# phylo42/IPK

Measured on AMD Instinct MI355X. Metric: scored phylo-k-mers/sec, higher is better.
Workload: dtype f32

## Files before the change

ipk_amd/csrc/ipkgpu.hip:

```cpp
#include <cstring>
#include <hip/hip_runtime.h>
#include <rocprim/rocprim.hpp>

#include <algorithm>
#include <cmath>
#include <cstdarg>
#include <cstdio>
#include <cstring>
#include <new>
#include <string>
#include <type_traits>
#include <unordered_map>
#include <memory>
#include <vector>

#include "../../include/ipkgpu.h"
#include "dcla_device.hpp"
#include "kernels_score.hpp"
#include "kernels_quad.hpp"
#include "kernels_compact.hpp"
#include "kernels_keymajor.hpp"
#include "kernels_reduce_pipe.hpp"
#include "kernels_filter.hpp"
#include "kernels_dbfile.hpp"
// ... 39 lines not shown
        if (!e) return -1;
        (void)hipEventRecord(e, stream);
        ev.push_back(e);
        return (int)ev.size() - 1;
    }
    double ms(int a, int b) const
    {
        float t = 0;
        if (a < 0 || b < 0 || hipEventElapsedTime(&t, ev[a], ev[b]) != hipSuccess) return 0;
        return t;
    }
};

}

struct ipkgpu_comm;
struct ipkgpu_ctx;
static void ipkgpu_comm_release(ipkgpu_ctx* ctx);
struct ipkgpu_ctx {
    int device = 0;
    ipkgpu_comm* comm = nullptr;
    hipStream_t stream = nullptr;
    std::string err;
    int64_t workspace_bytes = 0;
    int64_t opt_variant = 0;
    int64_t opt_flags = 0;
    int64_t opt_kmc_pass = 0;
    int64_t opt_slice = 0;
    uint64_t sliced_windows = 0;
    int64_t opt_prefix_mats = 0;
    int64_t opt_wg_chunks2 = 0;
    int64_t opt_rounds = 0;
    int64_t opt_pool_limit = 0;
    int64_t opt_pool_chunks = 0;
    DevBuf table, best, ovfq, counts, offsets, goff, idx, branch, scan_sums, scan_boff, tmp_a, tmp_b, tmp_c;
    DevBuf pool, desc, gbcnt, gboff, gbcur, clist, gm, tile_next;
    DevBuf ptrs;
    DevBuf sp_bits, sp_pops, sp_rank, sp_c16;
    void* h_spill[2] = {nullptr, nullptr}; hipEvent_t ev_spill[2] = {nullptr, nullptr}; size_t h_spill_cap = 0;
    size_t held = 0, held_peak = 0;
    int64_t budget = 0;
    size_t refused_need = 0;
    DevBuf mask;
    bool mask_valid = false;
    uint64_t mask_words = 0;
    bool table_compressed = false;
    DevBuf rank, vaddr, ucnt, qpack, xstart, pcounts;
    DevBuf seq, pvals, pvaddr, mrank, cursnap;
    DevBuf cvals, coff, croom;
    bool comp_own_vals = false;
    std::vector<uint32_t> h_branch;
    uint32_t comp_nb = 0, comp_stride = 0, comp_tbl = 0;
    double pairs_per_window = 0;
    double acc_main_ms = 0, acc_reduce_ms = 0;
    double acc_count_ms = 0, acc_write_ms = 0, acc_km_ms = 0;
    const char* main_kernel = "";
    std::vector<std::pair<void*, size_t>> free_blocks;
    std::unordered_map<void*, size_t> live_blocks;
    size_t cached_bytes = 0, cache_limit = 0;
    void* small = nullptr;
    void* h_up = nullptr; size_t h_up_cap = 0; hipEvent_t up_done = nullptr; bool up_pending = false;
    unsigned long long emitted_host = 0; bool emitted_fetched = false;
    uint32_t* h_rb = nullptr;
    EventPool events;
    bool spec_skip_wait = false;
    uint64_t pool_want_min = 0;
    struct Pending {
        bool active = false;
        std::unique_ptr<Stopwatch> sw; int ev_a = -1, ev_b = -1, ev_c = -1, ev_d = -1;
        uint64_t cap = 0, max_chunks = 0, windows = 0; uint32_t gb = 0; bool pool_ovf_ok = false, use_quad = false;
    } pend;
    uint64_t last_entries = 0; uint32_t last_gb = 0;
    double t_write_total = 0, t_write_device = 0, t_write_file = 0;
    int64_t opt_load_chunk = 0;
    double t_load[8] = {0, 0, 0, 0, 0, 0, 0, 0};
    double t_diff_ms = 0;
    DevBuf place_seq, place_off, place_out, place_tables, place_small, place_amb;
    int64_t opt_place_batch = 0;
    int64_t opt_place_lds = 0;
    int num_cu = 256;
};

struct ipkgpu_result {
    ipkgpu_ctx* ctx = nullptr;
    std::vector<uint32_t> group_ids;
    std::vector<uint64_t> offsets;
    uint64_t emitted = 0;
    uint32_t* d_keys = nullptr;
    float* d_scores = nullptr;
    uint32_t* d_positions = nullptr;
    size_t cap = 0;
    std::vector<uint32_t> h_keys;
    std::vector<float> h_scores;
    std::vector<uint32_t> h_positions;
    bool h_keys_ok = false, h_scores_ok = false, h_positions_ok = false;
    double t_total = 0, t_prefix = 0, t_score = 0, t_compact = 0, t_main = 0, t_reduce = 0;
    int score_launches = 0;
};

struct ipkgpu_parts {
    ipkgpu_ctx* ctx = nullptr;
    uint32_t n_owners = 1;
    uint64_t slots = 0;
    uint32_t* d_counts = nullptr;
    uint2* d_entries = nullptr;
    uint32_t* d_positions = nullptr;
// ... 1134 lines not shown
    p.mask = ctx->mask.as<uint32_t>(); p.mask_words = ctx->mask_words;
    if (ps.kind == PassKind::xp) {
        if (!ps.compress) {
            RC_TRY(ensure(ctx, ctx->table, (size_t)gb * pl.table_size * 4));
            p.table = ctx->table.p;
        }
        const int rc = score_batch_xp(ctx, pl, logp_dev, gb, p);
        return rc ? rc : check_capped(ctx, pl.k, p);
    }

    const bool pool_ovf_ok = gb < (1u << 22) && n_mats < (1u << 21) && pl.nwin < (1u << 21);
    bool s_compress = pool_ovf_ok && ps.compress;
    const uint32_t NBK = pl.geo.stream_nb, TBL = pl.geo.stream_tbl;
    const uint32_t SNW = use_quad ? pl.geo.quad_nw : pl.geo.stream_nw;
    const uint32_t STW = use_quad ? pl.geo.quad_tw : pl.geo.stream_tw;
    const uint32_t s_tiles_per_mat = (pl.nwin + STW - 1) / STW;
    auto pass1 = [&](const StreamParams& sp, uint32_t n_wg, bool count_only) {
        return with_sigma_k(ctx, pl.sigma, pl.k, [&](auto S_, auto K_) {
            if (!use_quad) return launch_stream_pass1<S_, K_>(ctx, sp, n_wg);
            return count_only ? launch_quad_pass1<S_, K_, true>(ctx, sp, n_wg, ps.layout) : launch_quad_pass1<S_, K_, false>(ctx, sp, n_wg, ps.layout);
        });
    };

    const uint64_t windows = (uint64_t)nb * pl.nwin;
    if (ctx->pairs_per_window <= 0) {
        const uint32_t n_s = std::min<uint32_t>(gb, std::max<uint32_t>(2, gb / 64));
        const uint32_t stride_g = gb / n_s;
        std::vector<uint32_t> sgm((size_t)n_s + 1, 0), slist;
        for (uint32_t j = 0; j < n_s; ++j) {
            const uint32_t g = j * stride_g;
            for (uint32_t m = gm[g]; m < gm[g + 1]; ++m) slist.push_back(gm[(size_t)gb + 1 + m]);
            sgm[j + 1] = (uint32_t)slist.size();
        }
        std::vector<uint32_t> both(sgm);
        both.insert(both.end(), slist.begin(), slist.end());
        RC_TRY(ensure(ctx, ctx->tmp_a, both.size() * 4));
        HIP_TRY(ctx, hipMemcpyAsync(ctx->tmp_a.p, both.data(), both.size() * 4, hipMemcpyHostToDevice, ctx->stream));
        HIP_TRY(ctx, hipMemsetAsync(p.emitted, 0, 8, ctx->stream));
        HIP_TRY(ctx, hipMemsetAsync(p.ovf_count, 0, 4, ctx->stream));
        StreamParams ss;
        ss.logp = logp_dev; ss.best = ctx->best.as<float>();
        ss.gm_off = ctx->tmp_a.as<uint32_t>(); ss.gm_list = ctx->tmp_a.as<uint32_t>() + n_s + 1;
        ss.sites = pl.sites; ss.nwin = pl.nwin; ss.tiles_per_mat = s_tiles_per_mat;
        ss.S = (uint32_t)std::max<uint64_t>(1, std::min<uint64_t>(s_tiles_per_mat, (uint64_t)ctx->num_cu * 4 / n_s));
        ss.eps = pl.eps;
        ss.pool = nullptr; ss.pool_cap = 0; ss.pool_next = nullptr; ss.desc = nullptr; ss.pool_ovf = nullptr; ss.pre_chunks = 0;
        ss.emitted = p.emitted; ss.ovf_queue = p.ovf_queue; ss.ovf_count = p.ovf_count; ss.mat_slot = p.mat_slot;
        ss.flags = 2u;
        RC_TRY(pass1(ss, n_s * ss.S, true));
        unsigned long long se = 0; uint32_t so = 0;
        HIP_TRY(ctx, hipMemcpyAsync(&se, p.emitted, 8, hipMemcpyDeviceToHost, ctx->stream));
        HIP_TRY(ctx, hipMemcpyAsync(&so, p.ovf_count, 4, hipMemcpyDeviceToHost, ctx->stream));
        HIP_TRY(ctx, hipStreamSynchronize(ctx->stream));
        const uint64_t s_windows = (uint64_t)slist.size() * pl.nwin;
        const double cap_pairs = 0.25 * (double)pl.geo.fast_cap * (double)pl.geo.fast_cap;
        if (s_windows) ctx->pairs_per_window = std::max(1.0, ((double)se + (double)so * cap_pairs) / (double)s_windows * 1.15);
    }
    const double ppw_est = ctx->pairs_per_window > 0 ? ctx->pairs_per_window : 256.0;
    if (!s_compress && pool_ovf_ok && ctx->opt_variant == 0 && pl.table_size >= (1u << 16) &&
        (double)windows * ppw_est < 0.5 * (double)gb * (double)pl.table_size)
        s_compress = true;
    if (!s_compress) {
        RC_TRY(ensure(ctx, ctx->table, (size_t)gb * pl.table_size * 4));
        p.table = ctx->table.p;
    }
    const size_t lds_bytes = use_quad ? pl.geo.quad_lds : pl.geo.stream_lds;
    const uint64_t wg_per_cu = std::max<uint64_t>(1, std::min<uint64_t>(32 / SNW, (160 * 1024) / std::max<size_t>(lds_bytes, 1)));
    const uint64_t slots = (uint64_t)ctx->num_cu * wg_per_cu;
    const uint32_t CH = chunk_pairs_rt(TBL);
    const uint64_t CHB = chunk_bytes_rt(TBL, ps.layout);
    const uint64_t expected_chunks = (uint64_t)((double)windows * ppw_est / CH);
#ifndef IPK_WG_CHUNKS2
#define IPK_WG_CHUNKS2 2
#endif
    const uint64_t wg_chunks2 = ctx->opt_wg_chunks2 > 0 ? (uint64_t)ctx->opt_wg_chunks2 : (uint64_t)IPK_WG_CHUNKS2;
    const uint64_t max_wg = std::max<uint64_t>(slots, expected_chunks * 2 / wg_chunks2 / ((uint64_t)SNW * NBK * SUB));
#ifndef IPK_ROUNDS
#define IPK_ROUNDS 8
#endif
    const uint64_t rounds = std::max<uint64_t>(1, std::min<uint64_t>(ctx->opt_rounds > 0 ? (uint64_t)ctx->opt_rounds : (uint64_t)IPK_ROUNDS, max_wg / slots));
    uint64_t S64 = std::max<uint64_t>(1, (slots * rounds) / gb);
    uint32_t S = (uint32_t)std::max<uint64_t>(1, std::min<uint64_t>(S64, s_tiles_per_mat));
    const uint32_t n_wg = gb * S;
    const uint64_t n_waves = (uint64_t)n_wg * SNW;
    const uint64_t n_gb = (uint64_t)gb * NBK;

    const size_t free_b = mem_free_bytes(ctx);
    uint64_t max_chunks = std::min<uint64_t>(0xFFFFFFF0ull, (uint64_t)(free_b + ctx->pool.cap + ctx->desc.cap) * 9 / 10 / (CHB + 8));
    if (ctx->opt_pool_limit > 0) max_chunks = std::min<uint64_t>(max_chunks, (uint64_t)ctx->opt_pool_limit / (CHB + 8));
    const double ppw = ctx->pairs_per_window > 0 ? ctx->pairs_per_window : 256.0;
    const uint64_t ovf_waves = (uint64_t)ctx->num_cu * 4 * OVF_NW;
    const uint64_t slack = 2 * (n_waves + ovf_waves) * NBK * SUB + (n_waves + ovf_waves) * ALLOC_BATCH + 1024;
    uint64_t want = (uint64_t)((double)windows * ppw * 1.25 / CH) + slack;
    {
        const uint64_t have = std::min<uint64_t>(std::max<uint64_t>(ctx->pool.cap / CHB, 1) - 1, ctx->desc.cap / 8);
        const uint64_t need = (uint64_t)((double)windows * ppw * 1.1 / CH) + (n_waves + ovf_waves) * (NBK * SUB + ALLOC_BATCH) + 1024;
        if (have >= need) want = have;
    }
    want = std::max<uint64_t>(want, ctx->pool_want_min);
    for (int attempt = 0; attempt < 6; ++attempt) {
        uint64_t cap = std::min<uint64_t>(want, max_chunks);
        const bool forced = attempt == 0 && ctx->opt_pool_chunks > 0 && ctx->pool_want_min == 0;
        if (forced) cap = (uint64_t)ctx->opt_pool_chunks;
        else if (cap < n_waves * NBK * SUB) {
            if (gb > 1) return IPKGPU_RETRY_SMALLER;
            return fail(ctx, IPKGPU_ERR_NOMEM, "the pair pool of ONE branch group does not fit device memory");
// ... 1476 lines not shown

std::string spill_block_path(const char* dir, uint32_t piece, uint32_t owner)
{
    char name[64];
    snprintf(name, sizeof name, "/p%u_b%u.blk", piece, owner);
    return std::string(dir) + name;
}

struct SpillFile {
    std::string path; ipkspill::Head head; uint64_t key_base = 0, entry_base = 0;
};

int spill_check_files(ipkgpu_ctx* ctx, uint32_t sigma, uint32_t k, uint32_t owner, uint32_t n_owners, const char* const* paths, uint32_t n_blocks,
                      uint64_t slots, std::vector<SpillFile>& files)
{
    files.resize(n_blocks);
    uint64_t keys = 0, entries = 0;
    for (uint32_t s = 0; s < n_blocks; ++s) {
        if (!paths[s]) return fail(ctx, IPKGPU_ERR_INVALID, "null path of block %u", s);
        SpillFile& f = files[s];
        f.path = paths[s];
        FILE* fh = fopen(paths[s], "rb");
        if (!fh) return fail(ctx, IPKGPU_ERR_INVALID, "cannot open spill block %s", paths[s]);
        struct stat st;
        const bool stat_ok = fstat(fileno(fh), &st) == 0;
        memset(&f.head, 0, sizeof f.head);
        const size_t got = fread(&f.head, 1, sizeof f.head, fh);
        fclose(fh);
        if (!stat_ok) return fail(ctx, IPKGPU_ERR_INVALID, "cannot stat spill block %s", paths[s]);
        const char* what = got < sizeof f.head ? "shorter than a block's head"
                                               : ipkspill::check_head(f.head, (uint64_t)st.st_size, sigma, k, n_owners, owner, slots);
        if (what) return fail(ctx, IPKGPU_ERR_INVALID, "spill block %s: %s", paths[s], what);
        f.key_base = keys; f.entry_base = entries;
        keys += f.head.n_keys; entries += f.head.n_entries;
    }
    return IPKGPU_OK;
}

}

extern "C" {

int ipkgpu_get_option(const ipkgpu_ctx* ctx, const char* name, int64_t* value)
{
    if (!ctx || !name || !value) return IPKGPU_ERR_INVALID;
    if (!strcmp(name, "workspace_bytes")) { *value = ctx->workspace_bytes; return IPKGPU_OK; }
    if (!strcmp(name, "device_budget_bytes")) { *value = ctx->budget; return IPKGPU_OK; }
    if (!strcmp(name, "last_refused_bytes")) { *value = (int64_t)ctx->refused_need; return IPKGPU_OK; }
    if (!strcmp(name, "slice_long_lists")) { *value = ctx->opt_slice; return IPKGPU_OK; }
    if (!strcmp(name, "db_load_chunk_bytes")) { *value = ctx->opt_load_chunk; return IPKGPU_OK; }
    if (!strcmp(name, "place_batch_queries")) { *value = ctx->opt_place_batch; return IPKGPU_OK; }
    if (!strcmp(name, "place_lds_branches")) { *value = ctx->opt_place_lds; return IPKGPU_OK; }
    if (!strcmp(name, "debug_sliced_windows")) { *value = (int64_t)ctx->sliced_windows; return IPKGPU_OK; }
    if (!strcmp(name, "debug_pool_bytes")) { *value = (int64_t)ctx->pool.cap; return IPKGPU_OK; }
    return IPKGPU_ERR_INVALID;
}

int ipkgpu_mem_stats(ipkgpu_ctx* ctx, uint64_t* held, uint64_t* held_peak, int reset_peak)
{
    if (!ctx) return IPKGPU_ERR_INVALID;
    if (held) *held = ctx->held;
    if (held_peak) *held_peak = ctx->held_peak;
    if (reset_peak) ctx->held_peak = ctx->held;
    return IPKGPU_OK;
}

int ipkgpu_parts_spill(ipkgpu_ctx* ctx, ipkgpu_parts* parts, const char* dir, uint32_t piece, uint64_t* bytes_written)
{
    if (!ctx) return IPKGPU_ERR_INVALID;
    if (!parts || parts->ctx != ctx || !dir) return fail(ctx, IPKGPU_ERR_INVALID, "bad argument");
    if (parts->d_positions) return fail(ctx, IPKGPU_ERR_INVALID, "positioned parts are not spilled: the on-disk build keeps no positions (as the reference's, db_builder.cpp:469)");
    if (parts->lead != 0) return fail(ctx, IPKGPU_ERR_INVALID, "key-range parts are not spilled: a key-range pass already bounds the device");
    if (!parts->d_counts || !parts->d_entries) return fail(ctx, IPKGPU_ERR_INVALID, "these parts' arrays have moved into a database");
    HIP_TRY(ctx, hipSetDevice(ctx->device));
    const uint32_t B = parts->n_owners;
    const uint64_t slots = parts->slots, W = ipkspill::bit_words(slots), n_words = (uint64_t)B * W;
    if (W > 0xFFFFFFFFull || (n_words + 3) / 4 > 0x7FFFFFFFull) return fail(ctx, IPKGPU_ERR_INVALID, "too many key slots to spill");
    RC_TRY(ensure(ctx, ctx->sp_bits, n_words * 8));
    RC_TRY(ensure(ctx, ctx->sp_pops, n_words * 4));
    RC_TRY(ensure(ctx, ctx->sp_rank, (n_words + 1) * 8));
    RC_TRY(ensure(ctx, ctx->goff, ((size_t)B + 1) * 8));
    uint32_t* d_big = small_at(ctx, SMALL_REC_BIG);
    HIP_TRY(ctx, hipMemsetAsync(d_big, 0, 4, ctx->stream));
    const uint32_t grid = (uint32_t)((n_words + 3) / 4);
    hipLaunchKernelGGL(spill_bits_kernel, dim3(grid), dim3(256), 0, ctx->stream, parts->d_counts, slots, W, n_words,
                       ctx->sp_bits.as<unsigned long long>(), ctx->sp_pops.as<uint32_t>(), d_big);
    HIP_TRY(ctx, hipGetLastError());
    RC_TRY(scan_u32(ctx, ctx->sp_pops.as<uint32_t>(), n_words, ctx->sp_rank.as<uint64_t>()));
    hipLaunchKernelGGL(gather_offsets_kernel, dim3((B + 1 + 255) / 256), dim3(256), 0, ctx->stream, ctx->sp_rank.as<uint64_t>(), (uint32_t)W, B + 1,
                       ctx->goff.as<uint64_t>());
    HIP_TRY(ctx, hipGetLastError());
    std::vector<uint64_t> key_base((size_t)B + 1);
    uint32_t h_big = 0;
    HIP_TRY(ctx, hipMemcpyAsync(key_base.data(), ctx->goff.p, ((size_t)B + 1) * 8, hipMemcpyDeviceToHost, ctx->stream));
    HIP_TRY(ctx, hipMemcpyAsync(&h_big, d_big, 4, hipMemcpyDeviceToHost, ctx->stream));
    HIP_TRY(ctx, hipStreamSynchronize(ctx->stream));
    if (h_big) return fail(ctx, IPKGPU_ERR_INVALID, "a key with more than %u entries in one piece: a spill block's counts are 16-bit (pieces of at most %u groups)",
                           ipkspill::COUNT_MAX, ipkspill::COUNT_MAX);
    RC_TRY(ensure(ctx, ctx->sp_c16, key_base[B] * 2));
    hipLaunchKernelGGL(spill_pack_kernel, dim3(grid), dim3(256), 0, ctx->stream, parts->d_counts, slots, W, n_words, ctx->sp_rank.as<uint64_t>(),
                       ctx->sp_c16.as<uint16_t>());
    HIP_TRY(ctx, hipGetLastError());

    uint64_t largest = 0;
    for (uint32_t o = 0; o < B; ++o)
        largest = std::max(largest, ipkspill::file_bytes(slots, key_base[o + 1] - key_base[o], parts->owner_off[o + 1] - parts->owner_off[o]));
// ... 163 lines not shown
```

ipk_amd/csrc/kernels_quad.hpp:

```cpp
#pragma once
#include "kernels_score.hpp"

namespace ipkgpu {

struct QuadNode { int J, H, TH, OFF; uint32_t F, CMUL; };
struct QuadStep { int H, A, B; };

template <int SIGMA, int K>
struct QuadGeo {
    using D = HalvesDD<SIGMA, K>;
    static constexpr int HL = D::HL, HR = D::HR, LA = D::LA, LB = D::LB, RA = D::RA, RB = D::RB;
    static constexpr bool OK = SIGMA == 4 && D::OK && LA >= 2 && LA <= 3 && LB >= 2 && LB <= 3 && RA >= 2 && RA <= 3 && RB >= 2 && RB <= 3;
    static constexpr uint32_t FLA = D::FLA, FLB = D::FLB, FRA = D::FRA, FRB = D::FRB;
    static constexpr uint32_t mulR = ipow(SIGMA, K - K / 2);
    static constexpr uint32_t CW = FLA + FLB + FRA + FRB;
    static constexpr int th_n(int h) { return h == 2 ? 3 : 5; }
    static constexpr int TH0 = 2, TH1 = TH0 + th_n(LA), TH2 = TH1 + th_n(LB), TH3 = TH2 + th_n(RA);
    static constexpr int TH_F = TH3 + th_n(RB);
    static constexpr int PADW = 1;
    static constexpr QuadNode node(int n)
    {
        return n == 0 ? QuadNode{0, LA, TH0, 0, FLA, 1u}
             : n == 1 ? QuadNode{LA, LB, TH1, (int)FLA, FLB, mulR}
             : n == 2 ? QuadNode{HL, RA, TH2, (int)(FLA + FLB), FRA, 1u}
                      : QuadNode{HL + RA, RB, TH3, (int)(FLA + FLB + FRA), FRB, 1u};
    }
    static constexpr int count_h(int h) { int c = 0; for (int n = 0; n < 4; ++n) c += node(n).H == h; return c; }
    static constexpr int nth_h(int h, int i) { for (int n = 0; n < 4; ++n) if (node(n).H == h) { if (i == 0) return n; --i; } return -1; }
    static constexpr int NS2 = (count_h(2) + 1) / 2, NS3 = (count_h(3) + 1) / 2, NSTEPS = NS2 + NS3;
    static constexpr QuadStep step(int s)
    {
        return s < NS2 ? QuadStep{2, nth_h(2, 2 * s), nth_h(2, 2 * s + 1)} : QuadStep{3, nth_h(3, 2 * (s - NS2)), nth_h(3, 2 * (s - NS2) + 1)};
    }
    static constexpr int step_of(int n) { for (int s = 0; s < NSTEPS; ++s) if (step(s).A == n || step(s).B == n) return s; return -1; }
    static constexpr int slot_of(int n) { return step(step_of(n)).B == n ? 1 : 0; }
    static constexpr int NS1 = (count_h(2) > 0 ? 1 : 0) + (count_h(3) > 0 ? 1 : 0);
    static constexpr int step1_h(int s) { return (s == 0 && count_h(2) > 0) ? 2 : 3; }
    static constexpr int step1_node(int s, int slot) { return nth_h(step1_h(s), slot); }
    static constexpr int step1_of(int n) { return node(n).H == 2 ? 0 : (count_h(2) > 0 ? 1 : 0); }
    static constexpr int slot1_of(int n) { int c = 0; for (int m = 0; m < n; ++m) c += node(m).H == node(n).H; return c; }
};

template <int SIGMA, int K, int TW>
struct QuadTile {
    static constexpr int TC = TW + K - 1 + QuadGeo<SIGMA, K>::PADW;
    static constexpr int COLS_F = TC * SIGMA;
    static constexpr int BEST_F = ((TC + 1 + 3) / 4) * 4;
    static constexpr int TH_FLOATS = (((TW + QuadGeo<SIGMA, K>::PADW) * QuadGeo<SIGMA, K>::TH_F + 3) / 4) * 4;
    static constexpr int HEAD_BYTES = (COLS_F + BEST_F + TH_FLOATS) * 4;
};

template <int SIGMA, int K, int CAP, bool ONEWIN = false>
constexpr uint32_t quad_wave_entries()
{
    using Q = QuadGeo<SIGMA, K>;
    return (ONEWIN ? 1 : 2) * Q::CW + Geo<SIGMA, Q::HL, CAP>::CAPH + Geo<SIGMA, Q::HR, CAP>::CAPH;
}

template <int J, int H>
__device__ __forceinline__ void quad_node_thresholds(const float* bs, float e, float* out)
{
    out[0] = e;
    if constexpr (H == 2) {
        out[1] = e - (bs[J + 2] - bs[J + 1]);
        out[2] = e - (bs[J + 1] - bs[J]);
    } else {
        static_assert(H == 3, "child nodes have 2 or 3 symbols");
        const float e_leaf = e - (bs[J + 3] - bs[J + 1]);
        const float e_pair = e - (bs[J + 1] - bs[J]);
        out[1] = e_leaf;
        out[2] = e_pair;
        out[3] = e_pair - (bs[J + 3] - bs[J + 2]);
        out[4] = e_pair - (bs[J + 2] - bs[J + 1]);
    }
}

template <int H>
__device__ __forceinline__ void quad_step(const float* cols, uint32_t base, bool valid, uint64_t vmask, const float* th, uint2* list,
                                          uint32_t l16, uint32_t slot, uint32_t lt16, uint32_t code16, uint32_t cmul, uint32_t& count)
{
    const float e = th[0];
    if constexpr (H == 2) {
        const float sl = cols[base + (l16 >> 2)], sr = cols[base + 4 + (l16 & 3u)];
        const float s = sl + sr;
        const bool c1 = sl > th[1], c2 = sr > th[2], c3 = s > e;
        const bool pass = valid & c1 & c2 & c3;
        const uint64_t m = vmask & ballot64(c1) & ballot64(c2) & ballot64(c3);
        const uint32_t x = (uint32_t)(m >> (16u * slot));
        const uint32_t pos = (uint32_t)__popc(x & lt16);
        if (pass) list[pos] = make_uint2(code16, __float_as_uint(s));
        count = (uint32_t)__popc(x & 0xFFFFu);
    } else {
        const float sj = cols[base + 4 + (l16 >> 2)], sl2 = cols[base + 8 + (l16 & 3u)];
        const float s2 = sj + sl2;
        const bool d1 = sj > th[3], d2 = sl2 > th[4], d3 = s2 > th[2];
        const bool okp = valid & d1 & d2 & d3;
        const uint64_t mp = vmask & ballot64(d1) & ballot64(d2) & ballot64(d3);
        uint32_t run = 0;
#pragma unroll
        for (int i = 0; i < 4; ++i) {
            const float si = cols[base + i];
            const float s = si + s2;
            const bool c1 = si > th[1], c2 = s > e;
            const bool pass = okp & c1 & c2;
            const uint64_t m = mp & ballot64(c1) & ballot64(c2);
            const uint32_t x = (uint32_t)(m >> (16u * slot));
            const uint32_t pos = (uint32_t)__popc(x & lt16) + run;
            if (pass) list[pos] = make_uint2(__umul24(cmul, (uint32_t)i * 16u) + code16, __float_as_uint(s));
            run += (uint32_t)__popc(x & 0xFFFFu);
        }
        count = run;
    }
}

__device__ __forceinline__ void pool_store(uint2* wave_base, uint32_t byte_off, uint2 val)
{
    const unsigned long long data = ((unsigned long long)val.y << 32) | val.x;
    asm volatile("global_store_dwordx2 %0, %1, %2" : : "v"(byte_off), "v"(data), "s"(wave_base) : "memory");
}
__device__ __forceinline__ uint32_t lshl3_add(uint32_t x, uint32_t y)
{
    uint32_t r;
    asm("v_lshl_add_u32 %0, %1, 3, %2" : "=v"(r) : "v"(x), "v"(y));
    return r;
}
__device__ __forceinline__ void pool_store_lanes(uint2* wave_base, uint32_t byte_off, uint2 val, uint64_t mask)
{
    const unsigned long long data = ((unsigned long long)val.y << 32) | val.x;
    IPK_ASSERT_FULL_EXEC();
    asm volatile("s_mov_b64 exec, %3\n\tglobal_store_dwordx2 %0, %1, %2\n\ts_mov_b64 exec, -1"
                 : : "v"(byte_off), "v"(data), "s"(wave_base), "s"(mask) : "memory");
}

__device__ __forceinline__ uint64_t pool_store_inside(uint2* wave_base, uint32_t byte_off, uint2 val, uint32_t v, uint64_t pass, uint32_t CH)
{
    const unsigned long long data = ((unsigned long long)val.y << 32) | val.x;
    uint64_t outside;
    IPK_ASSERT_FULL_EXEC();
    asm volatile("s_mov_b64 exec, %5\n\t"
                 "v_cmpx_gt_u32_e32 vcc, %6, %4\n\t"
                 "global_store_dwordx2 %1, %2, %3\n\t"
                 "s_andn2_b64 %0, %5, exec\n\t"
                 "s_mov_b64 exec, -1"
                 : "=&s"(outside) : "v"(byte_off), "v"(data), "s"(wave_base), "v"(v), "s"(pass), "s"(CH) : "memory", "vcc");
    return outside;
}


template <uint32_t SLOT_PLANE>
__device__ __forceinline__ void pool_store6(uint2* wave_base, uint32_t off4, uint32_t off2, uint2 val)
{
    static_assert(SLOT_PLANE < 4096, "the slot plane's offset must fit the store's immediate field");
    asm volatile("global_store_dword %0, %2, %4\n\tglobal_store_short %1, %3, %4 offset:%5"
                 : : "v"(off4), "v"(off2), "v"(val.y), "v"(val.x), "s"(wave_base), "n"(SLOT_PLANE) : "memory");
}
template <int SH>
__device__ __forceinline__ uint32_t lshl_add(uint32_t x, uint32_t y)
{
    uint32_t r;
    asm("v_lshl_add_u32 %0, %1, %3, %2" : "=v"(r) : "v"(x), "v"(y), "n"(SH));
    return r;
}
template <uint32_t SLOT_PLANE>
__device__ __forceinline__ uint64_t pool_store_inside6(uint2* wave_base, uint32_t off4, uint32_t off2, uint2 val, uint32_t v, uint64_t pass, uint32_t CH)
{
    static_assert(SLOT_PLANE < 4096, "the slot plane's offset must fit the store's immediate field");
    uint64_t outside;
    IPK_ASSERT_FULL_EXEC();
    asm volatile("s_mov_b64 exec, %7\n\t"
                 "v_cmpx_gt_u32_e32 vcc, %8, %6\n\t"
                 "global_store_dword %1, %3, %5\n\t"
                 "global_store_short %2, %4, %5 offset:%9\n\t"
                 "s_andn2_b64 %0, %7, exec\n\t"
                 "s_mov_b64 exec, -1"
                 : "=&s"(outside) : "v"(off4), "v"(off2), "v"(val.y), "v"(val.x), "s"(wave_base), "v"(v), "s"(pass), "s"(CH), "n"(SLOT_PLANE)
                 : "memory", "vcc");
    return outside;
// ... 92 lines not shown
    __device__ __forceinline__ void init(uint32_t wave_gid)
    {
        const uint32_t first = wave_gid * NB;
        const bool pre = p.pre_chunks != 0 && first + NB <= p.pre_chunks && first + NB <= p.pool_cap;
        for (uint32_t b = lane_id(); b < NB; b += 64)
            st[b] = pre ? ((unsigned long long)(first + b) << 32) : (((unsigned long long)NONE << 32) | (unsigned long long)CH);
    }
    __device__ __forceinline__ uint32_t roll_at(uint32_t b, uint32_t x)
    {
        const uint32_t lane = lane_id();
        if (chunk_next == chunk_end) {
            uint32_t first = 0;
            if (lane == 0) first = atomicAdd(p.pool_next, ALLOC_BATCH);
            chunk_next = (uint32_t)__builtin_amdgcn_readfirstlane((int)first);
            chunk_end = chunk_next + ALLOC_BATCH;
        }
        uint32_t nid = to_sgpr(chunk_next);
        chunk_next = nid + 1;
        if (nid >= p.pool_cap && lane == 0) atomicOr(p.pool_ovf, 1u);
        nid = min(nid, p.pool_cap);
        wave_lds_sync();
        const unsigned long long old = st[b];
        wave_lds_sync();
        if (lane == 0) {
            const uint32_t oid = (uint32_t)(old >> 32);
            if (oid < p.pool_cap) p.desc[oid] = ((unsigned long long)(g * NB + b) << 32) | (unsigned long long)x;
            st[b] = ((unsigned long long)nid << 32) | (unsigned long long)((uint32_t)old - x);
        }
        wave_lds_sync();
        return nid;
    }
    __device__ __forceinline__ void close()
    {
        wave_lds_sync();
        for (uint32_t b = lane_id(); b < NB; b += 64) {
            const unsigned long long s = st[b];
            const uint32_t id = (uint32_t)(s >> 32);
            if (id < p.pool_cap) p.desc[id] = ((unsigned long long)(g * NB + b) << 32) | (unsigned long long)min((uint32_t)s, CH);
        }
    }
};

__device__ __forceinline__ void store_pair_if_gt(unsigned long long& cursor, uint32_t x, float s, float eps)
{
    u32x2_t data; data.x = x; data.y = __float_as_uint(s);
    IPK_ASSERT_FULL_EXEC();
    asm volatile("v_cmpx_lt_f32_e32 vcc, %3, %2\n\t"
                 "global_store_dwordx2 %0, %1, off\n\t"
                 "v_lshl_add_u64 %0, %0, 0, 8\n\t"
                 "s_mov_b64 exec, -1"
                 : "+v"(cursor) : "v"(data), "v"(s), "s"(eps) : "vcc");
}

template <uint32_t MUL>
__device__ __forceinline__ uint32_t half_join_single(const uint2* A, const uint2* B, uint32_t nb, uint32_t total, float eps, uint2* out,
                                                     uint32_t lane, float lane_h)
{
    const float rn = __builtin_amdgcn_rcpf((float)nb);
    const uint32_t i = div_small(lane_h, rn), j = (uint32_t)(__mul24((int)i, -(int)nb) + (int)lane);
    const uint2 a = A[i], b = B[j];
    const float s = __uint_as_float(a.y) + __uint_as_float(b.y);
    const bool v = lane < total, c = s > eps;
    const uint64_t h = ballot64(v) & ballot64(c);
    if (v && c) out[mbcnt(h)] = make_uint2(a.x * MUL + b.x, __float_as_uint(s));
    return (uint32_t)__popcll(h);
}
template <uint32_t MUL>
__device__ __forceinline__ uint32_t half_join_rows(const uint2* A, uint32_t na, const uint2* B, uint32_t nb, float eps, uint2* out, uint32_t cap,
                                                   uint32_t lane, float lane_h)
{
    const float rn = __builtin_amdgcn_rcpf((float)nb);
    const uint32_t rps = to_sgpr(div_small(64.5f, rn));
    const uint32_t rsel = div_small(lane_h, rn), col = lane - __umul24(rsel, nb);
    const uint2 b = B[col];
    const float by = __uint_as_float(b.y);
    const uint2* ap = A + rsel;
    uint32_t n = 0;
    for (uint32_t i0 = 0; i0 < na; i0 += rps) {
        const uint2 a = ap[i0];
        const float s = __uint_as_float(a.y) + by;
        const bool live = lane < min(rps, na - i0) * nb, c = s > eps;
        const uint64_t m = ballot64(live) & ballot64(c);
        const uint32_t cnt = (uint32_t)__popcll(m);
        if (n + cnt > cap) return LIST_OVERFLOW;
        if (live && c) (out + n)[mbcnt(m)] = make_uint2(a.x * MUL + b.x, __float_as_uint(s));
        n += cnt;
    }
    return n;
}

template <int SIGMA, int K, int CAP, int TW, int NW, uint32_t TBL, bool COUNT_ONLY = false, bool ROWLANE = false, bool ONEWIN = false,
          PairLayout LAYOUT = PairLayout::PAIR8>
__global__ __launch_bounds__(NW * 64) void score_quad_kernel(StreamParams p)
{
    extern __shared__ __align__(16) unsigned char smem[];
    using Q = QuadGeo<SIGMA, K>;
    using QT = QuadTile<SIGMA, K, TW>;
    static_assert(Q::OK, "quad kernel: DNA k = 8..12");
    constexpr uint32_t T = ipow(SIGMA, K);
    constexpr uint32_t NB = (T + TBL - 1) / TBL;
    constexpr uint32_t CH = chunk_pairs<TBL>();
    constexpr uint32_t mulR = Q::mulR;
    static_assert(TBL % mulR == 0, "a row of the final join must stay inside one bucket");
    using CL = ChunkLayout<TBL, LAYOUT>;
    static_assert(!ROWLANE || LAYOUT == PairLayout::PAIR8, "the row-per-lane join writes 8-byte pairs");
    constexpr bool P6 = LAYOUT == PairLayout::PAIR6;
    constexpr uint32_t CAPL = Geo<SIGMA, Q::HL, CAP>::CAPH, CAPR = Geo<SIGMA, Q::HR, CAP>::CAPH;
    constexpr uint32_t WS = quad_wave_entries<SIGMA, K, CAP, ONEWIN>();
    constexpr uint32_t WPW = ONEWIN ? 1u : 2u;
    constexpr int NST = ONEWIN ? Q::NS1 : Q::NSTEPS;
    float* cols = reinterpret_cast<float*>(smem);
    float* best = cols + QT::COLS_F;
    float* thr = best + QT::BEST_F;
    uint2* scratch_all = reinterpret_cast<uint2*>(smem + QT::HEAD_BYTES);
    unsigned long long* state_all = reinterpret_cast<unsigned long long*>(scratch_all + (size_t)NW * WS);

    const uint32_t lane = lane_id();
    const uint32_t wave = (uint32_t)__builtin_amdgcn_readfirstlane((int)(threadIdx.x >> 6));
    const uint32_t g = blockIdx.x / p.S, seg = blockIdx.x - g * p.S;
    const uint32_t m0 = p.gm_off[g], nm = p.gm_off[g + 1] - m0;
    const uint32_t total_tiles = nm * p.tiles_per_mat;
    const uint32_t t_lo = (uint32_t)(((uint64_t)total_tiles * seg) / p.S);
    const uint32_t t_hi = (uint32_t)(((uint64_t)total_tiles * (seg + 1)) / p.S);

    uint2* child = scratch_all + (size_t)wave * WS;
    uint2* lp = child + WPW * Q::CW;
    uint2* rp = lp + CAPL;
    using Appender = std::conditional_t<ROWLANE, LaneAppender<NB, CH>, RowAppender<NB, CH, CL::PAIR_BYTES>>;
    Appender app{p, state_all + (size_t)wave * NB, g};
    app.init(blockIdx.x * NW + wave);
    unsigned long long emitted = 0;

    const uint32_t l16 = lane & 15u, slot = lane >> 4, half = ONEWIN ? 0u : lane >> 5, sb = slot & 1u;
    const uint32_t lt16 = (1u << l16) - 1u;
    const float lane_h = (float)lane + 0.5f;
    const float eps = p.eps;
    constexpr bool count_only = COUNT_ONLY;
    uint32_t st_j4[NST], st_th[NST], st_off[NST], st_cmul[NST], st_code[NST];
    bool st_on[NST];
#pragma unroll
    for (int s = 0; s < NST; ++s) {
        constexpr QuadNode none{0, 2, 0, 0, 0, 1u};
        if constexpr (ONEWIN) {
            QuadNode nd = none;
            bool on = false;
#pragma unroll
            for (int sl = 0; sl < 4; ++sl) {
                const int n = Q::step1_node(s, sl);
                if (n >= 0 && slot == (uint32_t)sl) { nd = Q::node(n); on = true; }
            }
            st_j4[s] = (uint32_t)nd.J * 4u; st_th[s] = (uint32_t)nd.TH; st_off[s] = (uint32_t)nd.OFF; st_cmul[s] = nd.CMUL;
            st_code[s] = l16 * st_cmul[s]; st_on[s] = on;
        } else {
            const QuadStep qs = Q::step(s);
            const QuadNode na = Q::node(qs.A), nb = qs.B >= 0 ? Q::node(qs.B) : none;
            st_j4[s] = sb ? (uint32_t)nb.J * 4u : (uint32_t)na.J * 4u;
            st_th[s] = sb ? (uint32_t)nb.TH : (uint32_t)na.TH;
            st_off[s] = (sb ? (uint32_t)nb.OFF : (uint32_t)na.OFF) + half * Q::CW;
            st_cmul[s] = sb ? nb.CMUL : na.CMUL;
            st_code[s] = l16 * st_cmul[s];
            st_on[s] = sb ? qs.B >= 0 : true;
        }
    }

    __shared__ uint32_t sh_tile;
    const bool draw = p.tile_next != nullptr;
    uint32_t t = t_lo, t_end = t_hi;
    if (draw) { t = seg; t_end = total_tiles; }
    while (t < t_end) {
        const uint32_t q = t / p.tiles_per_mat, tile = t - q * p.tiles_per_mat;
        const uint32_t mat = p.gm_list[m0 + q];
        const uint32_t t0 = tile * TW;
        const uint32_t nw = min((uint32_t)TW, p.nwin - t0);
        const uint32_t ncol = nw + K - 1;
        __syncthreads();
        uint32_t t_drawn = 0;
        if (draw && threadIdx.x == 0) t_drawn = atomicAdd(&p.tile_next[g], 1u);
        {
            const float4* src = reinterpret_cast<const float4*>(p.logp + ((size_t)mat * p.sites + t0) * SIGMA);
            float4* dst = reinterpret_cast<float4*>(cols);
            const uint32_t n4 = ncol * (SIGMA / 4);
            for (uint32_t i = threadIdx.x; i < n4; i += NW * 64) dst[i] = src[i];
            const float* bsrc = p.best + (size_t)mat * (p.sites + 1) + t0;
            for (uint32_t i = threadIdx.x; i <= ncol; i += NW * 64) best[i] = bsrc[i];
        }
        if (draw && threadIdx.x == 0) sh_tile = t_drawn;
        __syncthreads();
        for (uint32_t w = threadIdx.x; w < nw; w += NW * 64) {
            const float* bs = best + w;
            float* o = thr + w * Q::TH_F;
            const float eps_l = eps - (bs[K] - bs[Q::HL]);
            const float eps_r = eps - (bs[Q::HL] - bs[0]);
            o[0] = eps_l; o[1] = eps_r;
            quad_node_thresholds<0, Q::LA>(bs, eps_l - (bs[Q::HL] - bs[Q::LA]), o + Q::node(0).TH);
            quad_node_thresholds<Q::LA, Q::LB>(bs, eps_l - (bs[Q::LA] - bs[0]), o + Q::node(1).TH);
            quad_node_thresholds<Q::HL, Q::RA>(bs, eps_r - (bs[K] - bs[Q::HL + Q::RA]), o + Q::node(2).TH);
            quad_node_thresholds<Q::HL + Q::RA, Q::RB>(bs, eps_r - (bs[Q::HL + Q::RA] - bs[Q::HL]), o + Q::node(3).TH);
        }
        __syncthreads();

        const uint32_t npair = (nw + WPW - 1) / WPW;
        const float* thw = thr + __umul24(wave * WPW + half, (uint32_t)Q::TH_F);
        for (uint32_t pr = wave; pr < npair; pr += NW, thw += WPW * NW * Q::TH_F) {
            const uint32_t wq = pr * WPW;
            const uint32_t wl = wq + half;
            const bool wvalid = wl < nw;
            uint32_t counts[3] = {0, 0, 0};
            wave_lds_sync();
            auto run_step = [&](auto S) {
                constexpr int s = decltype(S)::value;
                if constexpr (s < NST) {
                    const bool valid = wvalid && st_on[s];
                    const uint64_t vmask = ballot64(valid);
                    const uint32_t base = wl * 4 + st_j4[s];
                    constexpr int H = ONEWIN ? Q::step1_h(s) : Q::step(s < Q::NSTEPS ? s : 0).H;
                    quad_step<H>(cols, base, valid, vmask, thw + st_th[s], child + st_off[s], l16, slot, lt16, st_code[s], st_cmul[s], counts[s]);
                }
            };
            run_step(std::integral_constant<int, 0>{});
            run_step(std::integral_constant<int, 1>{});
            run_step(std::integral_constant<int, 2>{});
            wave_lds_sync();
            const uint32_t nwp = min(WPW, nw - wq);

#pragma unroll 1
            for (uint32_t gw = 0; gw < nwp; ++gw) {
                const uint32_t w = wq + gw;
                constexpr int so0 = ONEWIN ? Q::step1_of(0) : Q::step_of(0), so1 = ONEWIN ? Q::step1_of(1) : Q::step_of(1);
                constexpr int so2 = ONEWIN ? Q::step1_of(2) : Q::step_of(2), so3 = ONEWIN ? Q::step1_of(3) : Q::step_of(3);
                constexpr int sl0 = ONEWIN ? Q::slot1_of(0) : Q::slot_of(0), sl1 = ONEWIN ? Q::slot1_of(1) : Q::slot_of(1);
                constexpr int sl2 = ONEWIN ? Q::slot1_of(2) : Q::slot_of(2), sl3 = ONEWIN ? Q::slot1_of(3) : Q::slot_of(3);
                const uint32_t wbase = ONEWIN ? 0u : gw * 32u;
                const uint32_t nla = (uint32_t)__builtin_amdgcn_readlane((int)counts[so0], (int)(wbase + sl0 * 16));
                const uint32_t nlb = (uint32_t)__builtin_amdgcn_readlane((int)counts[so1], (int)(wbase + sl1 * 16));
                const uint32_t nra = (uint32_t)__builtin_amdgcn_readlane((int)counts[so2], (int)(wbase + sl2 * 16));
                const uint32_t nrb = (uint32_t)__builtin_amdgcn_readlane((int)counts[so3], (int)(wbase + sl3 * 16));
                if (nla * nlb * nra * nrb == 0) continue;
                const uint2* cw = child + gw * Q::CW;
                const uint2 *la = cw + Q::node(0).OFF, *lb = cw + Q::node(1).OFF, *ra = cw + Q::node(2).OFF, *rb = cw + Q::node(3).OFF;
                const float eps_l = thr[w * Q::TH_F], eps_r = thr[w * Q::TH_F + 1];
                const uint32_t tl = nla * nlb, tr = nra * nrb;
                uint32_t nL, nR;
                constexpr bool SLICE = ROWLANE;
                constexpr uint32_t SAFE_L = CAPL / Q::FLB, SAFE_R = CAPR / Q::FRB;
                static_assert(SAFE_L >= 1 && SAFE_R >= 1, "a slice of one row of the first child must fit the list");
                const bool one_step = tl <= 64 && tr <= 64;
                uint32_t sla = nla, sra = nra, ia = 0, ir = 0;
                bool keep_l = false;
                for (;;) {
                wave_lds_sync();
                if (one_step) {
                    const float rnl = __builtin_amdgcn_rcpf((float)nlb), rnr = __builtin_amdgcn_rcpf((float)nrb);
                    const uint32_t il = div_small(lane_h, rnl), jl = (uint32_t)(__mul24((int)il, -(int)nlb) + (int)lane);
                    const uint32_t ir = div_small(lane_h, rnr), jr = (uint32_t)(__mul24((int)ir, -(int)nrb) + (int)lane);
                    const uint2 a0 = la[il], b0 = lb[jl], a1 = ra[ir], b1 = rb[jr];
                    const float s0 = __uint_as_float(a0.y) + __uint_as_float(b0.y);
                    const float s1 = __uint_as_float(a1.y) + __uint_as_float(b1.y);
                    const bool v0 = lane < tl, v1 = lane < tr, c0 = s0 > eps_l, c1 = s1 > eps_r;
                    const bool p0 = v0 && c0, p1 = v1 && c1;
                    const uint64_t h0 = ballot64(v0) & ballot64(c0), h1 = ballot64(v1) & ballot64(c1);
                    if (p0) lp[mbcnt(h0)] = make_uint2(a0.x * (Q::FLB * mulR) + b0.x, __float_as_uint(s0));
                    if (p1) rp[mbcnt(h1)] = make_uint2(a1.x * Q::FRB + b1.x, __float_as_uint(s1));
                    nL = (uint32_t)__popcll(h0); nR = (uint32_t)__popcll(h1);
                } else {
                    if constexpr (!ROWLANE) {
                        nL = (uint32_t)__builtin_amdgcn_readfirstlane((int)(tl <= 64 ? half_join_single<Q::FLB * mulR>(la, lb, nlb, tl, eps_l, lp, lane, lane_h)
                                                                                       : half_join_rows<Q::FLB * mulR>(la, nla, lb, nlb, eps_l, lp, CAPL, lane, lane_h)));
                        nR = nL == LIST_OVERFLOW || nL == 0 ? nL
                           : (uint32_t)__builtin_amdgcn_readfirstlane((int)(tr <= 64 ? half_join_single<Q::FRB>(ra, rb, nrb, tr, eps_r, rp, lane, lane_h)
                                                                                      : half_join_rows<Q::FRB>(ra, nra, rb, nrb, eps_r, rp, CAPR, lane, lane_h)));
                    } else {
                    if (!keep_l)
                        nL = (uint32_t)__builtin_amdgcn_readfirstlane((int)join_to_list(la + ia, min(sla, nla - ia), lb, nlb, eps_l, Q::FLB * mulR, lp, CAPL));
                    if constexpr (SLICE) {
                        if (nL == LIST_OVERFLOW) { sla = SAFE_L; continue; }
                    }
                    nR = nL == LIST_OVERFLOW || nL == 0 ? nL : (uint32_t)__builtin_amdgcn_readfirstlane((int)join_to_list(ra + ir, min(sra, nra - ir), rb, nrb, eps_r, Q::FRB, rp, CAPR));
                    }
                    if constexpr (SLICE) {
                        if (nR == LIST_OVERFLOW) { sra = SAFE_R; keep_l = true; continue; }
                    } else if (nL == LIST_OVERFLOW || nR == LIST_OVERFLOW) {
                        if (lane == 0) {
                            const uint32_t qi = atomicAdd(p.ovf_count, 1u);
                            p.ovf_queue[qi] = ((unsigned long long)mat << 32) | (unsigned long long)(t0 + w);
                        }
                        __builtin_amdgcn_wave_barrier();
                        break;
                    }
                }
                if (nL != 0 && nR != 0) {
                wave_lds_sync();
                if (p.flags & 4u) emitted += nL + nR;
                else
                if constexpr (ROWLANE) {
                    constexpr uint32_t CB = 64;
                    static_assert(CB <= CH, "row-per-lane join: a run must fit a chunk");
                    for (uint32_t ib = 0; ib < nL; ib += 64) {
                        const uint2 a = lp[ib + lane];
                        const bool rv = ib + lane < nL;
                        const float ay = rv ? __uint_as_float(a.y) : -__builtin_inff();
                        const uint32_t bk = a.x / TBL;
                        for (uint32_t jb = 0; jb < nR; jb += CB) {
                            const uint32_t nc = min(CB, nR - jb);
                            const uint2* rj = rp + jb;
                            uint32_t cnt = 0;
                            if constexpr (count_only) {
                                for (uint32_t j = 0; j < nc; ++j) emitted += (uint32_t)__popcll(ballot64(ay + __uint_as_float(rj[j].y) > eps));
                            } else {
                                auto count8 = [&](auto NC, uint32_t j0, uint32_t& n, float e) {
                                    constexpr uint32_t N = decltype(NC)::value;
                                    float by[N];
#pragma unroll
                                    for (uint32_t u = 0; u < N; ++u) by[u] = __uint_as_float(rj[j0 + u].y);
#pragma unroll
                                    for (uint32_t u = 0; u < N; ++u) {
                                        const float sj = ay + by[u];
                                        asm("v_cmp_lt_f32_e32 vcc, %2, %1\n\tv_addc_co_u32_e32 %0, vcc, 0, %0, vcc" : "+v"(n) : "v"(sj), "s"(e) : "vcc");
                                    }
                                };
                                uint32_t j0 = 0;
                                for (; j0 + 8 <= nc; j0 += 8) count8(std::integral_constant<uint32_t, 8>{}, j0, cnt, eps);
                                if (j0 + 4 <= nc) { count8(std::integral_constant<uint32_t, 4>{}, j0, cnt, eps); j0 += 4; }
// ... 160 lines not shown
```

Baseline: 142.7 billion.

## Precompute per-step LDS pointers and use masked-exec LDS stores in quad join

The per-step column, threshold and list addresses are now computed once outside the window loop, so each iteration only adds a window offset. Predicated list appends are replaced by inline-asm ds_write_b64 stores that set exec to the ballot mask, and the four H=3 sub-step counts are combined with perm and bcnt. This aims to cut VALU and branch overhead in the hot first-level join. It also adds debug counters for the count pass. The cost is more live pointer registers and hand-written exec manipulation, which may hurt occupancy or correctness if the exec assumptions fail.

```diff
diff --git a/ipk_amd/csrc/ipkgpu.hip b/ipk_amd/csrc/ipkgpu.hip
--- a/ipk_amd/csrc/ipkgpu.hip
+++ b/ipk_amd/csrc/ipkgpu.hip
@@ -115,6 +115,8 @@
     std::vector<uint32_t> h_branch;
     uint32_t comp_nb = 0, comp_stride = 0, comp_tbl = 0;
     double pairs_per_window = 0;
+    uint64_t count_pass_pairs = 0;
+    uint64_t count_pass_queued = 0;
     double acc_main_ms = 0, acc_reduce_ms = 0;
     double acc_count_ms = 0, acc_write_ms = 0, acc_km_ms = 0;
     const char* main_kernel = "";
@@ -1355,6 +1357,7 @@
         HIP_TRY(ctx, hipMemcpyAsync(&se, p.emitted, 8, hipMemcpyDeviceToHost, ctx->stream));
         HIP_TRY(ctx, hipMemcpyAsync(&so, p.ovf_count, 4, hipMemcpyDeviceToHost, ctx->stream));
         HIP_TRY(ctx, hipStreamSynchronize(ctx->stream));
+        ctx->count_pass_pairs = se; ctx->count_pass_queued = so;
         const uint64_t s_windows = (uint64_t)slist.size() * pl.nwin;
         const double cap_pairs = 0.25 * (double)pl.geo.fast_cap * (double)pl.geo.fast_cap;
         if (s_windows) ctx->pairs_per_window = std::max(1.0, ((double)se + (double)so * cap_pairs) / (double)s_windows * 1.15);
@@ -2937,6 +2940,8 @@
     if (!strcmp(name, "place_batch_queries")) { *value = ctx->opt_place_batch; return IPKGPU_OK; }
     if (!strcmp(name, "place_lds_branches")) { *value = ctx->opt_place_lds; return IPKGPU_OK; }
     if (!strcmp(name, "debug_sliced_windows")) { *value = (int64_t)ctx->sliced_windows; return IPKGPU_OK; }
+    if (!strcmp(name, "debug_count_pass_pairs")) { *value = (int64_t)ctx->count_pass_pairs; return IPKGPU_OK; }
+    if (!strcmp(name, "debug_count_pass_queued")) { *value = (int64_t)ctx->count_pass_queued; return IPKGPU_OK; }
     if (!strcmp(name, "debug_pool_bytes")) { *value = (int64_t)ctx->pool.cap; return IPKGPU_OK; }
     return IPKGPU_ERR_INVALID;
 }
diff --git a/ipk_amd/csrc/kernels_quad.hpp b/ipk_amd/csrc/kernels_quad.hpp
--- a/ipk_amd/csrc/kernels_quad.hpp
+++ b/ipk_amd/csrc/kernels_quad.hpp
@@ -75,54 +75,81 @@
     }
 }
 
-template <int H>
-__device__ __forceinline__ void quad_step(const float* cols, uint32_t base, bool valid, uint64_t vmask, const float* th, uint2* list,
-                                          uint32_t l16, uint32_t slot, uint32_t lt16, uint32_t code16, uint32_t cmul, uint32_t& count)
-{
-    const float e = th[0];
-    if constexpr (H == 2) {
-        const float sl = cols[base + (l16 >> 2)], sr = cols[base + 4 + (l16 & 3u)];
-        const float s = sl + sr;
-        const bool c1 = sl > th[1], c2 = sr > th[2], c3 = s > e;
-        const bool pass = valid & c1 & c2 & c3;
-        const uint64_t m = vmask & ballot64(c1) & ballot64(c2) & ballot64(c3);
-        const uint32_t x = (uint32_t)(m >> (16u * slot));
-        const uint32_t pos = (uint32_t)__popc(x & lt16);
-        if (pass) list[pos] = make_uint2(code16, __float_as_uint(s));
-        count = (uint32_t)__popc(x & 0xFFFFu);
-    } else {
-        const float sj = cols[base + 4 + (l16 >> 2)], sl2 = cols[base + 8 + (l16 & 3u)];
-        const float s2 = sj + sl2;
-        const bool d1 = sj > th[3], d2 = sl2 > th[4], d3 = s2 > th[2];
-        const bool okp = valid & d1 & d2 & d3;
-        const uint64_t mp = vmask & ballot64(d1) & ballot64(d2) & ballot64(d3);
-        uint32_t run = 0;
-#pragma unroll
-        for (int i = 0; i < 4; ++i) {
-            const float si = cols[base + i];
-            const float s = si + s2;
-            const bool c1 = si > th[1], c2 = s > e;
-            const bool pass = okp & c1 & c2;
-            const uint64_t m = mp & ballot64(c1) & ballot64(c2);
-            const uint32_t x = (uint32_t)(m >> (16u * slot));
-            const uint32_t pos = (uint32_t)__popc(x & lt16) + run;
-            if (pass) list[pos] = make_uint2(__umul24(cmul, (uint32_t)i * 16u) + code16, __float_as_uint(s));
-            run += (uint32_t)__popc(x & 0xFFFFu);
-        }
-        count = run;
-    }
-}
-
-__device__ __forceinline__ void pool_store(uint2* wave_base, uint32_t byte_off, uint2 val)
-{
-    const unsigned long long data = ((unsigned long long)val.y << 32) | val.x;
-    asm volatile("global_store_dwordx2 %0, %1, %2" : : "v"(byte_off), "v"(data), "s"(wave_base) : "memory");
-}
 __device__ __forceinline__ uint32_t lshl3_add(uint32_t x, uint32_t y)
 {
     uint32_t r;
     asm("v_lshl_add_u32 %0, %1, 3, %2" : "=v"(r) : "v"(x), "v"(y));
     return r;
+}
+__device__ __forceinline__ uint32_t lds_addr(const void* p)
+{
+    typedef const char __attribute__((address_space(3)))* lds_ptr;
+    return (uint32_t)(uintptr_t)(lds_ptr)p;
+}
+template <uint32_t IMM = 0>
+__device__ __forceinline__ void lds_put8_lanes(uint32_t addr, uint32_t x, uint32_t y, uint64_t mask)
+{
+    static_assert(IMM < 65536 && IMM % 8 == 0, "the offset must fit the store's 16-bit field");
+    u32x2_t data; data.x = x; data.y = y;
+    IPK_ASSERT_FULL_EXEC();
+    asm volatile("s_mov_b64 exec, %2\n\tds_write_b64 %0, %1 offset:%3\n\ts_mov_b64 exec, -1" : : "v"(addr), "v"(data), "s"(mask), "n"(IMM) : "memory");
+}
+__device__ __forceinline__ uint2 lds_entry(uint32_t base, uint32_t j)
+{
+    typedef const u32x2_t __attribute__((address_space(3)))* lds_pair_ptr;
+    uint32_t a;
+    asm("v_lshl_add_u32 %0, %1, 3, %2" : "=v"(a) : "v"(j), "s"(base));
+    const u32x2_t v = *(lds_pair_ptr)(uintptr_t)a;
+    return make_uint2(v.x, v.y);
+}
+__device__ __forceinline__ uint32_t bcnt_add(uint32_t x, uint32_t acc)
+{
+    uint32_t r;
+    asm("v_bcnt_u32_b32 %0, %1, %2" : "=v"(r) : "v"(x), "v"(acc));
+    return r;
+}
+
+template <int H>
+__device__ __forceinline__ void quad_step(const float* ca, const float* cb, const float* ci, uint64_t vmask, const float* th, uint32_t list,
+                                          uint32_t sh16, uint32_t lt16, uint32_t lt16w, uint32_t code16, uint32_t cmul, uint32_t& count)
+{
+    const float e = th[0];
+    if constexpr (H == 2) {
+        const float sl = ca[0], sr = cb[0];
+        const float s = sl + sr;
+        const bool c1 = sl > th[1], c2 = sr > th[2], c3 = s > e;
+        const uint64_t m = vmask & ballot64(c1) & ballot64(c2) & ballot64(c3);
+        const uint32_t x = (uint32_t)(m >> sh16);
+        lds_put8_lanes(lshl3_add((uint32_t)__popc(x & lt16), list), code16, __float_as_uint(s), m);
+        count = (uint32_t)__popc(x & 0xFFFFu);
+    } else {
+        const float sj = ca[0], sl2 = cb[0];
+        const float s2 = sj + sl2;
+        const bool d1 = sj > th[3], d2 = sl2 > th[4], d3 = s2 > th[2];
+        const uint64_t mp = vmask & ballot64(d1) & ballot64(d2) & ballot64(d3);
+        float s[4]; uint64_t m[4]; uint32_t x[4];
+#pragma unroll
+        for (int i = 0; i < 4; ++i) {
+            const float si = ci[i];
+            s[i] = si + s2;
+            const bool c1 = si > th[1], c2 = s[i] > e;
+            m[i] = mp & ballot64(c1) & ballot64(c2);
+            x[i] = (uint32_t)(m[i] >> sh16);
+        }
+        const uint32_t y01 = __builtin_amdgcn_perm(x[1], x[0], 0x05040100u);
+        const uint32_t y23 = __builtin_amdgcn_perm(x[3], x[2], 0x05040100u);
+        const uint32_t n01 = (uint32_t)__popc(y01);
+        const uint32_t pos[4] = {(uint32_t)__popc(x[0] & lt16), (uint32_t)__popc(y01 & lt16w), bcnt_add(x[2] & lt16, n01), bcnt_add(y23 & lt16w, n01)};
+#pragma unroll
+        for (int i = 0; i < 4; ++i) lds_put8_lanes(lshl3_add(pos[i], list), __umul24(cmul, (uint32_t)i * 16u) + code16, __float_as_uint(s[i]), m[i]);
+        count = bcnt_add(y23, n01);
+    }
+}
+
+__device__ __forceinline__ void pool_store(uint2* wave_base, uint32_t byte_off, uint2 val)
+{
+    const unsigned long long data = ((unsigned long long)val.y << 32) | val.x;
+    asm volatile("global_store_dwordx2 %0, %1, %2" : : "v"(byte_off), "v"(data), "s"(wave_base) : "memory");
 }
 __device__ __forceinline__ void pool_store_lanes(uint2* wave_base, uint32_t byte_off, uint2 val, uint64_t mask)
 {
@@ -321,17 +348,16 @@
                  : "+v"(cursor) : "v"(data), "v"(s), "s"(eps) : "vcc");
 }
 
-template <uint32_t MUL>
-__device__ __forceinline__ uint32_t half_join_single(const uint2* A, const uint2* B, uint32_t nb, uint32_t total, float eps, uint2* out,
+template <uint32_t MUL, uint32_t OUT_OFF>
+__device__ __forceinline__ uint32_t half_join_single(const uint2* A, const uint2* B, uint32_t nb, uint32_t total, float eps, uint32_t out,
                                                      uint32_t lane, float lane_h)
 {
     const float rn = __builtin_amdgcn_rcpf((float)nb);
     const uint32_t i = div_small(lane_h, rn), j = (uint32_t)(__mul24((int)i, -(int)nb) + (int)lane);
-    const uint2 a = A[i], b = B[j];
+    const uint2 a = A[i], b = lds_entry(lds_addr(B), j);
     const float s = __uint_as_float(a.y) + __uint_as_float(b.y);
-    const bool v = lane < total, c = s > eps;
-    const uint64_t h = ballot64(v) & ballot64(c);
-    if (v && c) out[mbcnt(h)] = make_uint2(a.x * MUL + b.x, __float_as_uint(s));
+    const uint64_t h = (~0ull >> (64u - total)) & ballot64(s > eps);
+    lds_put8_lanes<OUT_OFF>(out + (mbcnt(h) << 3), a.x * MUL + b.x, __float_as_uint(s), h);
     return (uint32_t)__popcll(h);
 }
 template <uint32_t MUL>
@@ -395,41 +421,57 @@
     uint2* child = scratch_all + (size_t)wave * WS;
     uint2* lp = child + WPW * Q::CW;
     uint2* rp = lp + CAPL;
+    constexpr uint32_t LP_OFF = WPW * Q::CW * 8u, RP_OFF = LP_OFF + CAPL * 8u;
+    const uint32_t child_a = lds_addr(child);
     using Appender = std::conditional_t<ROWLANE, LaneAppender<NB, CH>, RowAppender<NB, CH, CL::PAIR_BYTES>>;
     Appender app{p, state_all + (size_t)wave * NB, g};
     app.init(blockIdx.x * NW + wave);
     unsigned long long emitted = 0;
 
     const uint32_t l16 = lane & 15u, slot = lane >> 4, half = ONEWIN ? 0u : lane >> 5, sb = slot & 1u;
-    const uint32_t lt16 = (1u << l16) - 1u;
+    const uint32_t lt16 = (1u << l16) - 1u, lt16w = 0xFFFFu | (lt16 << 16), sh16 = slot * 16u;
     const float lane_h = (float)lane + 0.5f;
     const float eps = p.eps;
     constexpr bool count_only = COUNT_ONLY;
-    uint32_t st_j4[NST], st_th[NST], st_off[NST], st_cmul[NST], st_code[NST];
-    bool st_on[NST];
+    constexpr bool CB_FROM_CA = NST > 2;
+    const uint32_t cb_ca = 4u + (l16 & 3u) - (l16 >> 2);
+    const float *st_ca[NST], *st_cb[NST], *st_ci[NST], *st_thp[NST];
+    uint32_t st_list[NST];
+    uint32_t st_cmul[NST], st_code[NST];
+    uint64_t ST_ON[NST];
 #pragma unroll
     for (int s = 0; s < NST; ++s) {
         constexpr QuadNode none{0, 2, 0, 0, 0, 1u};
+        uint32_t j4, tho, off;
         if constexpr (ONEWIN) {
             QuadNode nd = none;
-            bool on = false;
+            uint64_t on = 0;
 #pragma unroll
             for (int sl = 0; sl < 4; ++sl) {
                 const int n = Q::step1_node(s, sl);
-                if (n >= 0 && slot == (uint32_t)sl) { nd = Q::node(n); on = true; }
+                if (n >= 0) on |= 0xFFFFull << (16 * sl);
+                if (n >= 0 && slot == (uint32_t)sl) nd = Q::node(n);
             }
-            st_j4[s] = (uint32_t)nd.J * 4u; st_th[s] = (uint32_t)nd.TH; st_off[s] = (uint32_t)nd.OFF; st_cmul[s] = nd.CMUL;
-            st_code[s] = l16 * st_cmul[s]; st_on[s] = on;
+            j4 = (uint32_t)nd.J * 4u; tho = (uint32_t)nd.TH; off = (uint32_t)nd.OFF; st_cmul[s] = nd.CMUL;
+            ST_ON[s] = on;
         } else {
             const QuadStep qs = Q::step(s);
             const QuadNode na = Q::node(qs.A), nb = qs.B >= 0 ? Q::node(qs.B) : none;
-            st_j4[s] = sb ? (uint32_t)nb.J * 4u : (uint32_t)na.J * 4u;
-            st_th[s] = sb ? (uint32_t)nb.TH : (uint32_t)na.TH;
-            st_off[s] = (sb ? (uint32_t)nb.OFF : (uint32_t)na.OFF) + half * Q::CW;
+            j4 = sb ? (uint32_t)nb.J * 4u : (uint32_t)na.J * 4u;
+            tho = sb ? (uint32_t)nb.TH : (uint32_t)na.TH;
+            off = (sb ? (uint32_t)nb.OFF : (uint32_t)na.OFF) + half * Q::CW;
             st_cmul[s] = sb ? nb.CMUL : na.CMUL;
-            st_code[s] = l16 * st_cmul[s];
-            st_on[s] = sb ? qs.B >= 0 : true;
-        }
+            ST_ON[s] = qs.B >= 0 ? ~0ull : 0x0000FFFF0000FFFFull;
+        }
+        st_code[s] = l16 * st_cmul[s];
+        const int H = ONEWIN ? Q::step1_h(s) : Q::step(s < Q::NSTEPS ? s : 0).H;
+        const float* c0 = cols + (wave * WPW + half) * 4u + j4;
+        st_ci[s] = c0;
+        st_ca[s] = c0 + (H == 2 ? 0u : 4u) + (l16 >> 2);
+        st_cb[s] = c0 + (H == 2 ? 4u : 8u) + (l16 & 3u);
+        st_thp[s] = thr + (wave * WPW + half) * (uint32_t)Q::TH_F + tho;
+        st_list[s] = child_a + off * 8u;
+        asm("" : "+v"(st_list[s]));
     }
 
     __shared__ uint32_t sh_tile;
@@ -469,21 +511,20 @@
         __syncthreads();
 
         const uint32_t npair = (nw + WPW - 1) / WPW;
-        const float* thw = thr + __umul24(wave * WPW + half, (uint32_t)Q::TH_F);
-        for (uint32_t pr = wave; pr < npair; pr += NW, thw += WPW * NW * Q::TH_F) {
+        for (uint32_t pr = wave; pr < npair; pr += NW) {
             const uint32_t wq = pr * WPW;
-            const uint32_t wl = wq + half;
-            const bool wvalid = wl < nw;
+            const uint32_t wo = wq - wave * WPW;
+            const uint64_t wmask = ONEWIN || wq + 1 < nw ? ~0ull : 0xFFFFFFFFull;
             uint32_t counts[3] = {0, 0, 0};
             wave_lds_sync();
             auto run_step = [&](auto S) {
                 constexpr int s = decltype(S)::value;
                 if constexpr (s < NST) {
-                    const bool valid = wvalid && st_on[s];
-                    const uint64_t vmask = ballot64(valid);
-                    const uint32_t base = wl * 4 + st_j4[s];
                     constexpr int H = ONEWIN ? Q::step1_h(s) : Q::step(s < Q::NSTEPS ? s : 0).H;
-                    quad_step<H>(cols, base, valid, vmask, thw + st_th[s], child + st_off[s], l16, slot, lt16, st_code[s], st_cmul[s], counts[s]);
+                    const uint32_t co = wo * 4u, to = wo * (uint32_t)Q::TH_F;
+                    const float* ca = st_ca[s] + co;
+                    quad_step<H>(ca, CB_FROM_CA ? ca + cb_ca : st_cb[s] + co, st_ci[s] + co, wmask & ST_ON[s], st_thp[s] + to, st_list[s], sh16, lt16, lt16w,
+                                 st_code[s], st_cmul[s], counts[s]);
                 }
             };
             run_step(std::integral_constant<int, 0>{});
@@ -522,21 +563,19 @@
                     const float rnl = __builtin_amdgcn_rcpf((float)nlb), rnr = __builtin_amdgcn_rcpf((float)nrb);
                     const uint32_t il = div_small(lane_h, rnl), jl = (uint32_t)(__mul24((int)il, -(int)nlb) + (int)lane);
                     const uint32_t ir = div_small(lane_h, rnr), jr = (uint32_t)(__mul24((int)ir, -(int)nrb) + (int)lane);
-                    const uint2 a0 = la[il], b0 = lb[jl], a1 = ra[ir], b1 = rb[jr];
+                    const uint2 a0 = la[il], b0 = lds_entry(lds_addr(lb), jl), a1 = ra[ir], b1 = lds_entry(lds_addr(rb), jr);
                     const float s0 = __uint_as_float(a0.y) + __uint_as_float(b0.y);
                     const float s1 = __uint_as_float(a1.y) + __uint_as_float(b1.y);
-                    const bool v0 = lane < tl, v1 = lane < tr, c0 = s0 > eps_l, c1 = s1 > eps_r;
-                    const bool p0 = v0 && c0, p1 = v1 && c1;
-                    const uint64_t h0 = ballot64(v0) & ballot64(c0), h1 = ballot64(v1) & ballot64(c1);
-                    if (p0) lp[mbcnt(h0)] = make_uint2(a0.x * (Q::FLB * mulR) + b0.x, __float_as_uint(s0));
-                    if (p1) rp[mbcnt(h1)] = make_uint2(a1.x * Q::FRB + b1.x, __float_as_uint(s1));
+                    const uint64_t h0 = (~0ull >> (64u - tl)) & ballot64(s0 > eps_l), h1 = (~0ull >> (64u - tr)) & ballot64(s1 > eps_r);
+                    lds_put8_lanes<LP_OFF>(child_a + (mbcnt(h0) << 3), a0.x * (Q::FLB * mulR) + b0.x, __float_as_uint(s0), h0);
+                    lds_put8_lanes<RP_OFF>(child_a + (mbcnt(h1) << 3), a1.x * Q::FRB + b1.x, __float_as_uint(s1), h1);
                     nL = (uint32_t)__popcll(h0); nR = (uint32_t)__popcll(h1);
                 } else {
                     if constexpr (!ROWLANE) {
-                        nL = (uint32_t)__builtin_amdgcn_readfirstlane((int)(tl <= 64 ? half_join_single<Q::FLB * mulR>(la, lb, nlb, tl, eps_l, lp, lane, lane_h)
+                        nL = (uint32_t)__builtin_amdgcn_readfirstlane((int)(tl <= 64 ? half_join_single<Q::FLB * mulR, LP_OFF>(la, lb, nlb, tl, eps_l, child_a, lane, lane_h)
                                                                                        : half_join_rows<Q::FLB * mulR>(la, nla, lb, nlb, eps_l, lp, CAPL, lane, lane_h)));
                         nR = nL == LIST_OVERFLOW || nL == 0 ? nL
-                           : (uint32_t)__builtin_amdgcn_readfirstlane((int)(tr <= 64 ? half_join_single<Q::FRB>(ra, rb, nrb, tr, eps_r, rp, lane, lane_h)
+                           : (uint32_t)__builtin_amdgcn_readfirstlane((int)(tr <= 64 ? half_join_single<Q::FRB, RP_OFF>(ra, rb, nrb, tr, eps_r, child_a, lane, lane_h)
                                                                                       : half_join_rows<Q::FRB>(ra, nra, rb, nrb, eps_r, rp, CAPR, lane, lane_h)));
                     } else {
                     if (!keep_l)
```

Measured after the change: 145.6 billion (median of 6 runs). 2.0% higher.
